# posgraph/coupe.DVSG

Measured on AMD Instinct MI355X. Metric: stabilized frames/sec (1280x720 RGB), higher is better.
Workload: dtype f32

## Files before the change

coupe/dvsg_amd/csrc/cnn_kernels.h:

```cpp
#pragma once
#include <type_traits>

#include "common.h"

namespace dvsg {

enum Precision { kF32 = 0, kF16 = 1, kF32S = 2, kF32X = 3 };
constexpr size_t elem_size(int prec) { return prec == kF16 ? 2 : 4; }
enum ConvMath { kMathF32, kMathF32S, kMathF32X, kMathF16Pairs, kMathF16Plain };
constexpr Precision storage_of(ConvMath m) { return m == kMathF32S ? kF32S : m == kMathF16Pairs || m == kMathF16Plain ? kF16 : kF32; }
constexpr ConvMath math_of(int prec, bool pairs) {
  return prec == kF16 ? (pairs ? kMathF16Pairs : kMathF16Plain) : prec == kF32S ? kMathF32S : prec == kF32X ? kMathF32X : kMathF32;
}
constexpr size_t elem_size(ConvMath m) { return elem_size((int)storage_of(m)); }
static_assert(storage_of(kMathF32) == kF32 && storage_of(kMathF32X) == kF32 && storage_of(kMathF32S) == kF32S &&
              storage_of(kMathF16Pairs) == kF16 && storage_of(kMathF16Plain) == kF16, "ConvMath -> storage format");
static_assert(math_of(kF32, false) == kMathF32 && math_of(kF32, true) == kMathF32 && math_of(kF32S, false) == kMathF32S &&
              math_of(kF32S, true) == kMathF32S && math_of(kF32X, false) == kMathF32X && math_of(kF32X, true) == kMathF32X &&
              math_of(kF16, true) == kMathF16Pairs && math_of(kF16, false) == kMathF16Plain, "(Precision, pairs) -> ConvMath");
static_assert(elem_size(kMathF32) == 4 && elem_size(kMathF32S) == 4 && elem_size(kMathF32X) == 4 &&
              elem_size(kMathF16Pairs) == 2 && elem_size(kMathF16Plain) == 2, "ConvMath -> bytes per tensor element");

struct ConvWeights {
  const void *rows = nullptr, *packed = nullptr, *packed_a = nullptr, *packed_h = nullptr;
// ... 86 lines not shown
  const int rec[6] = {family, nw, to, src, bands, quads};
  for (int i = 0; i < 6; ++i) g_last_root_kernel[i] = rec[i];
}
enum Conv1SrcKind { kSrcWindow = 0, kSrcRingF32 = 1, kSrcRingU8 = 2 };
constexpr int kSrcAligned = 1;
constexpr int kSrcKindShift = 1;
constexpr int kSrcMasked = 8;
constexpr int conv1_src(int kind, bool aligned, bool masked) {
  return (kind << kSrcKindShift) | (aligned ? kSrcAligned : 0) | (masked ? kSrcMasked : 0);
}
struct Conv1Src {
  const void *base;
  const int *table;
  int n_pool;
  const float *mask = nullptr;
};
struct Conv1Weights {
  const float *f32;
  const _Float16 *f16;
  const _Float16 *pieces;
  const unsigned short *x3;
  const float *bias;
};
int launch_conv1(int out_prec, const Conv1Src &src, int src_kind, const Conv1Weights &wt, void *y, int B, int H, int W, int Ho,
                 int Wo, int cin, hipStream_t s);
int prepare_rootconv();
int prepare_root_band();

int launch_maxpool(int prec, const void *x, void *y, int B, int H, int W, int C, int Ho, int Wo, int pad_top,
                   int pad_left, hipStream_t s);

constexpr int kPoolSplits = 8;
int launch_avgpool_partial(int prec, const void *x, float *part, int B, int HW, int C, hipStream_t s);

int launch_f16_to_f32(const void *x, float *y, size_t n, hipStream_t s);
int launch_p_to_f32(const void *x, float *y, size_t n, hipStream_t s);
int launch_f32_to_p(const float *x, void *y, size_t n, hipStream_t s);

constexpr int kDenseSplits = 8;
int launch_dense(const float *xin, int s_in, const float *bias_in, float scale_in, int lrelu_in,
                 const float *W, float *out_part, int B, int K, int N, hipStream_t s);
int launch_dense_finalize(const float *part, int s_in, float scale, const float *bias, float *out, int B,
                          int N, hipStream_t s);

}
```

coupe/dvsg_amd/csrc/common.h:

```cpp
#pragma once
#include <hip/hip_runtime.h>

#include <cstdarg>
#include <cstdio>

#include "../../../include/dvsg_amd.h"

namespace dvsg {

char *error_buffer();
int fail(int status, const char *fmt, ...) __attribute__((format(printf, 2, 3)));

inline hipStream_t as_stream(void *s) { return reinterpret_cast<hipStream_t>(s); }

inline int check_launch(const char *what) {
  hipError_t e = hipGetLastError();
  if (e != hipSuccess) return fail(DVSG_ERR_HIP, "%s: %s", what, hipGetErrorString(e));
  return DVSG_OK;
}

#define DVSG_REQUIRE(cond, ...)                                  \
  do {                                                           \
    if (!(cond)) return ::dvsg::fail(DVSG_ERR_INVALID_ARG, __VA_ARGS__); \
  } while (0)
// ... 26 lines not shown
int tps_render_impl(const double *winv_cols, const float *coord, const float *F_t, const uint8_t *src, int B, int H, int W,
                    int P, int channel_flip, float *T, float *out_f32, uint8_t *out_u8, int u8_W, int u8_x0, void *stream,
                    const float *zoom = nullptr, int render_filter = DVSG_RENDER_BILINEAR ,
                    int render_border = DVSG_BORDER_BLACK ,
                    RenderShape shape = RenderShape() );
int tps_render_nv12_check(const float *F_t, const uint8_t *y, const uint8_t *uv, size_t pitch, size_t frame_stride, int n,
                          int H, int W, const float *T, const uint8_t *out_y, const uint8_t *out_uv, size_t out_pitch,
                          size_t out_frame_stride, const char *fn = "dvsg_tps_render_nv12");
int tps_render_p010_check(const uint8_t *y, const uint8_t *uv, size_t pitch, size_t frame_stride, int n, int W,
                          const uint8_t *out_y, const uint8_t *out_uv, size_t out_pitch, size_t out_frame_stride, const char *fn);
int tps_render_nv12_impl(const double *winv_cols, const float *coord, const float *F_t, const uint8_t *y, const uint8_t *uv,
                         size_t pitch, size_t frame_stride, int n, int H, int W, int P, float *T, uint8_t *out_y,
                         uint8_t *out_uv, size_t out_pitch, size_t out_frame_stride, void *stream,
                         const float *zoom = nullptr, int render_filter = DVSG_RENDER_BILINEAR,
                         int render_border = DVSG_BORDER_BLACK, RenderShape shape = RenderShape(),
                         int surface_format = DVSG_SURFACE_NV12);
int tps_coverage_impl(const char *fn, const float *coord, long coord_bstride, const float *T, const float *zoom, int B, int P,
                      int src_H, int src_W, int out_h, int out_w, int32_t *n_border, int32_t *key_min, void *workspace,
                      size_t workspace_bytes, void *stream);

struct DebugOptions {
  int conv_variant = 0;
  int conv1_variant = 0;
  int wide16_min_tiles = 128;
  int wide16_packed = 1;
  int wide16_arows = 1;
  int wide16_hreuse = 1;
  int fused_hreuse = 1;
  int fuse_conv = 1;
  int fuse_shortcut = 1;
  int concat_sc = 1;
  int x3_conv1 = 1;
  int x3_fuse = 3;
  int f16_split = 1;
  int f16_pair_mask = 0xFFFF;
  int flow_tiled = 1;
  int flow_rounds = 4;
  int warp_xcd = 0;
};
extern DebugOptions g_opt;

inline int ceil_div(long a, long b) { return (int)((a + b - 1) / b); }

__device__ __forceinline__ uint8_t to_u8(double x) {
  const double d = x * 255.0;
  return d >= 255.0 ? (uint8_t)255 : (d > 0.0 ? (uint8_t)(int)d : (uint8_t)0);
// ... 36 lines not shown
```

coupe/dvsg_amd/csrc/conv1_pool.hip:

```cpp
#include <cstdint>
#include <type_traits>
#include <utility>

#include "cnn_device.h"
#include "cnn_kernels.h"

namespace dvsg {
namespace {

constexpr int C1_TILE = 128;
constexpr int C1_SEG_PAD = 5488;
constexpr int C1_WELEMS = 64 * kConv1Ld;
constexpr int C1_LDC = 68;

template <int NT, int GROUPS, bool ALIGNED, bool MASKED = false>
struct Conv1Row {
  static constexpr bool kRing = false;
  typedef float floatx4_u __attribute__((ext_vector_type(4), aligned(4)));
  floatx4 nmean[GROUPS];
  long idx[GROUPS];
  unsigned col_ok, full;
  bool fast;
  struct Data {
    floatx4 reg[GROUPS];
// ... 448 lines not shown
  __syncthreads();
  TO *yrow = y + (((size_t)b * Ho + ho) * Wo + wo0) * 64 + 4 * (tid & 15);
  conv1_tile_out<NT / 16>(Cs, conv1_tile_bias(bias, tid), tid, wo0, Wo,
                          [&](int row, float4 v) __attribute__((always_inline)) { store4(yrow + (size_t)row * 64, v); });
#ifdef DVSG_STAMPS
  if (tid == 0 && blockIdx.x < 65536) {
    unsigned long long *o = g_c1_stamps + (size_t)blockIdx.x * 8;
    const unsigned long long t_end = C1_STAMP();
    o[0] = st[0]; o[1] = st[1]; o[2] = st[2]; o[3] = st[3]; o[4] = st[4];
    o[5] = t_loop_end - t_begin;
    o[6] = t_end - t_begin;
    o[7] = __builtin_amdgcn_s_memrealtime() - r_begin;
  }
#endif
}

constexpr int RB_NT = 512;
constexpr int RB_IN4 = (C1_SEG_PAD / 4 + RB_NT - 1) / RB_NT;
constexpr int RB_WLOADS = (C1_WELEMS / 4 + RB_NT - 1) / RB_NT;
constexpr int RB_SLOTS = 3;
constexpr size_t RB_LDS = sizeof(float) * (size_t)(2 * C1_WELEMS + RB_SLOTS * C1_SEG_PAD);
static_assert(RB_LDS <= 160 * 1024, "the band kernel's LDS must fit a CU");

template <int SRC>
__global__ __launch_bounds__(RB_NT) __attribute__((amdgpu_waves_per_eu(2, 2)))
void root_band_kernel(const Conv1Src src, const float *__restrict__ wt1, const float *__restrict__ bias,
                      float *__restrict__ y, int H, int W, int Ho, int Wo, int wtiles, int bands, int ppb, int nbig) {
  constexpr int NT = RB_NT, MI = 2;
  static_assert(C1_TILE * C1_LDC <= C1_WELEMS, "epilogue tile must fit in a weight buffer");
  extern __shared__ __attribute__((aligned(16))) float rb_lds[];
  float *const w_s = rb_lds;
  float *const in_s = rb_lds + 2 * C1_WELEMS;
  const int tid = threadIdx.x;
  const int lane = tid & 63, wave = tid >> 6;
  const int wr = wave >> 2, wm = (wave >> 1) & 1, wn = wave & 1;
  const int r = lane & 31, h = lane >> 5;

  const Conv1Tile tile = conv1_tile(wtiles, bands);
  const int b = tile.b, band = tile.ho, wo0 = tile.wo0;
  const int pairs = (Ho + 1) / 2;
  const int p0 = band * ppb - (band > nbig ? band - nbig : 0);
  const int p1 = min(p0 + (band < nbig ? ppb : ppb - 1), pairs);
  if (p0 >= p1) return;

#ifdef DVSG_STAMPS
  unsigned long long st[8] = {0, 0, 0, 0, 0, 0, 0, 0};
  const unsigned long long t_begin = C1_STAMP(), r_begin = __builtin_amdgcn_s_memrealtime();
#endif
  typedef typename Conv1RowSel<NT, RB_IN4, SRC>::type Row;
  Row row;
  row.init(src, tid, b, wo0, H, W, C1_SEG_PAD);
  if constexpr (Row::kRing) {
    for (int e = tid; e < RB_SLOTS * C1_SEG_PAD; e += NT) in_s[e] = 0.f;
    __syncthreads();
  }
  typename Row::Data rd[3];
  floatx4 w_reg[RB_WLOADS];
  auto load_w = [&](int kh) __attribute__((always_inline)) {
    const floatx4 *wsrc = reinterpret_cast<const floatx4 *>(wt1 + (size_t)kh * C1_WELEMS);
#pragma unroll
    for (int i = 0; i < RB_WLOADS; ++i) {
      const int q = tid + NT * i;
      w_reg[i] = wsrc[q < C1_WELEMS / 4 ? q : 0];
    }
  };
  auto put_w = [&](int i, float *dst) __attribute__((always_inline)) {
    const int q = tid + NT * i;
    if (q < C1_WELEMS / 4) reinterpret_cast<floatx4 *>(dst)[q] = w_reg[i];
  };
  auto put_row = [&](const typename Row::Data &d, float *slot) __attribute__((always_inline)) {
    if constexpr (Row::kRing) {
      row.scatter(d, [&](int e, float v) __attribute__((always_inline)) { slot[e] = v; });
    } else {
#pragma unroll
      for (int i = 0; i < RB_IN4; ++i) {
        const int q = tid + NT * i;
        const floatx4 v = row.scaled(d, i);
        if (q < C1_SEG_PAD / 4) reinterpret_cast<floatx4 *>(slot)[q] = v;
      }
    }
  };
  auto load_first = [&](int ho_) __attribute__((always_inline)) {
#pragma unroll
    for (int i = 0; i < 3; ++i) row.load(rd[i], 2 * ho_ - 3 + i);
    load_w(0);
  };
#ifdef DVSG_STAMPS
  st[0] = C1_STAMP() - t_begin;
#endif
  load_first(2 * p0);

  for (int p = p0; p < p1; ++p) {
    const int ho = 2 * p;
#ifdef DVSG_STAMPS
    const unsigned long long f0 = C1_STAMP();
#endif
#pragma unroll
    for (int i = 0; i < RB_WLOADS; ++i) put_w(i, w_s);
#pragma unroll
    for (int i = 0; i < 3; ++i) {
      __builtin_amdgcn_sched_barrier(0);
      put_row(rd[i], in_s + i * C1_SEG_PAD);
    }
    __builtin_amdgcn_sched_barrier(0);
    floatx16 acc[MI], acc2[MI];
#pragma unroll
    for (int mi = 0; mi < MI; ++mi)
#pragma unroll
      for (int q = 0; q < 16; ++q) acc[mi][q] = acc2[mi][q] = 0.f;
#ifdef DVSG_STAMPS
    const unsigned long long f1 = C1_STAMP();
    __syncthreads();
    st[2] += f1 - f0;
    st[3] += C1_STAMP() - f1;
#else
    __syncthreads();
#endif

    int s_up = 0;
    for (int t = 0; t < 7; ++t) {
#ifdef DVSG_STAMPS
      const unsigned long long s3 = C1_STAMP();
#endif
      if (t < 6) {
        row.load(rd[0], 2 * ho + t);
        load_w(t + 1);
      }
#ifdef DVSG_STAMPS
      st[4] += C1_STAMP() - s3;
#endif
      __builtin_amdgcn_sched_barrier(0);
      const int s_lo = s_up == 0 ? 2 : s_up - 1;
      const float *a0 = in_s + (wr ? s_lo : s_up) * C1_SEG_PAD + 2 * kConv1Cin * (wm * 32 * MI + r) + 2 * h;
      const float *bp = w_s + (t & 1) * C1_WELEMS + (wn * 32 + r) * kConv1Ld + 2 * h;
      float *w_next = w_s + ((t + 1) & 1) * C1_WELEMS;
      constexpr int STEPS = kConv1Kpad / 4, PAIRS = (STEPS + 1) / 2;
      constexpr int WPUT0 = PAIRS / 2;
      float2 va[2][2][MI], vb[2][2];
      auto read_pair = [&](int slot, int g) __attribute__((always_inline)) {
#pragma unroll
        for (int j = 0; j < 2; ++j) {
          if (2 * g + j >= STEPS) break;
#pragma unroll
          for (int mi = 0; mi < MI; ++mi)
            va[slot][j][mi] = *reinterpret_cast<const float2 *>(a0 + mi * (2 * kConv1Cin * 32) + 4 * (2 * g + j));
          vb[slot][j] = *reinterpret_cast<const float2 *>(bp + 4 * (2 * g + j));
        }
      };
      read_pair(0, 0);
#pragma unroll
      for (int g = 0; g < PAIRS; ++g) {
        if (g + 1 < PAIRS) read_pair((g + 1) & 1, g + 1);
        if (g >= WPUT0 && g < WPUT0 + RB_WLOADS) put_w(g - WPUT0, w_next);
        __builtin_amdgcn_sched_barrier(0);
#pragma unroll
        for (int j = 0; j < 2; ++j) {
          if (2 * g + j >= STEPS) break;
#pragma unroll
          for (int mi = 0; mi < MI; ++mi) acc[mi] = mfma32(va[g & 1][j][mi].x, vb[g & 1][j].x, acc[mi]);
#pragma unroll
          for (int mi = 0; mi < MI; ++mi) acc2[mi] = mfma32(va[g & 1][j][mi].y, vb[g & 1][j].y, acc2[mi]);
        }
        __builtin_amdgcn_sched_barrier(0);
      }
      if (t < 6) {
#ifdef DVSG_STAMPS
        const unsigned long long s0 = C1_STAMP();
        __syncthreads();
        const unsigned long long s1 = C1_STAMP();
        put_row(rd[0], in_s + s_up * C1_SEG_PAD);
        const unsigned long long s2 = C1_STAMP();
        __syncthreads();
        st[1] += s1 - s0;
        st[2] += s2 - s1;
        st[3] += C1_STAMP() - s2;
#else
        __syncthreads();
        put_row(rd[0], in_s + s_up * C1_SEG_PAD);
        __syncthreads();
#endif
      }
      s_up = s_up == 2 ? 0 : s_up + 1;
    }

#ifdef DVSG_STAMPS
    const unsigned long long e0 = C1_STAMP();
#endif
    __syncthreads();
    float *Cs = w_s + wr * C1_WELEMS;
#pragma unroll
    for (int mi = 0; mi < MI; ++mi)
      C1_TILE_PUT(Cs, wm * 32 * MI + mi * 32, wn * 32, acc[mi][q] + acc2[mi][q]);
    __builtin_amdgcn_sched_barrier(0);
    if (p + 1 < p1) load_first(ho + 2);
    int tid_e = tid;
    asm volatile("" : "+v"(tid_e));
    const float4 b4 = conv1_tile_bias(bias, tid_e);
    __builtin_amdgcn_sched_barrier(0);
    __syncthreads();
#pragma unroll
    for (int j = 0; j < 2; ++j) {
      if (ho + j >= Ho) break;
      float *yrow = y + (((size_t)b * Ho + ho + j) * Wo + wo0) * 64 + 4 * (tid_e & 15);
      conv1_tile_out<NT / 16>(w_s + j * C1_WELEMS, b4, tid_e, wo0, Wo,
                              [&](int row_, float4 v) __attribute__((always_inline)) { store4(yrow + (size_t)row_ * 64, v); });
    }
    __syncthreads();
#ifdef DVSG_STAMPS
    st[5] += C1_STAMP() - e0;
#endif
  }
#ifdef DVSG_STAMPS
  if (tid == 0 && blockIdx.x < 65536) {
    unsigned long long *o = g_c1_stamps + (size_t)blockIdx.x * 8;
    o[0] = st[0]; o[1] = st[1]; o[2] = st[2]; o[3] = st[3]; o[4] = st[4]; o[5] = st[5];
    o[6] = C1_STAMP() - t_begin;
    o[7] = __builtin_amdgcn_s_memrealtime() - r_begin;
  }
#endif
}

struct PPieces {};

constexpr int rootconv_seg(int cin) { return C1_RING_PX * rootconv_pitch(cin) + 4; }
constexpr int rootconv_wstage(int cin) { return 64 * rootconv_ld(cin) > C1_TILE * C1_LDC ? 64 * rootconv_ld(cin) : C1_TILE * C1_LDC; }
constexpr size_t rootconv_lds_bytes(int cin) { return sizeof(float) * (size_t)(rootconv_wstage(cin) + rootconv_seg(cin)); }
static_assert(rootconv_lds_bytes(3 * kRootMaxFrames) <= 160 * 1024, "the largest window must fit one workgroup's LDS");

template <typename TO, int SRC>
__global__ __launch_bounds__(256)
void rootconv_kernel(const Conv1Src src, const float *__restrict__ wt1, const float *__restrict__ bias, void *__restrict__ y,
                     int H, int W, int Ho, int Wo, int wtiles, int cin) {
  constexpr int NT = 256, MI = 2;
  constexpr int kKind = SRC >> kSrcKindShift & 3;
  constexpr bool kMasked = (SRC & kSrcMasked) != 0;
  static_assert(SRC >= 0 && SRC < 16 && kKind <= kSrcRingU8, "no such conv1 source");
  extern __shared__ __attribute__((aligned(16))) float rc_lds[];
  const int S = cin / 3, pitch = rootconv_pitch(cin), ldw = rootconv_ld(cin), steps = rootconv_kpad(cin) / 4;
  const int welems = 64 * ldw, seg = rootconv_seg(cin);
  float *w_s = rc_lds;
  float *in_s = rc_lds + rootconv_wstage(cin);
  const int tid = threadIdx.x;
// ... 1088 lines not shown
}

template <int S>
using SrcC = std::integral_constant<int, S>;
template <bool MASKED_TOO, typename F>
bool with_conv1_src(int src, F &&f) {
  auto is = [&](auto c) { return src == c && (f(c), true); };
  if (is(SrcC<conv1_src(kSrcWindow, false, false)>{}) || is(SrcC<conv1_src(kSrcWindow, true, false)>{}) ||
      is(SrcC<conv1_src(kSrcRingF32, false, false)>{}) || is(SrcC<conv1_src(kSrcRingF32, true, false)>{}) ||
      is(SrcC<conv1_src(kSrcRingU8, false, false)>{}) || is(SrcC<conv1_src(kSrcRingU8, true, false)>{}))
    return true;
  if constexpr (MASKED_TOO)
    return is(SrcC<conv1_src(kSrcWindow, false, true)>{}) || is(SrcC<conv1_src(kSrcWindow, true, true)>{}) ||
           is(SrcC<conv1_src(kSrcRingF32, false, true)>{}) || is(SrcC<conv1_src(kSrcRingF32, true, true)>{}) ||
           is(SrcC<conv1_src(kSrcRingU8, false, true)>{}) || is(SrcC<conv1_src(kSrcRingU8, true, true)>{});
  return false;
}

}

int g_last_root_kernel[kRootKernelFields] = {-1, -1, -1, -1, -1, -1, -1, -1, -1};

int launch_conv1(int out_prec, const Conv1Src &src, int src_kind, const Conv1Weights &wt, void *y, int B, int H, int W, int Ho,
                 int Wo, int cin, hipStream_t s) {
  const float *const wt1 = wt.f32, *const bias = wt.bias;
  const _Float16 *const wt1h = wt.f16, *const wt1s = wt.pieces;
  const unsigned short *const wt1x = wt.x3;
  DVSG_REQUIRE(cin % 3 == 0 && cin >= 3 && cin <= 3 * kRootMaxFrames, "conv1: %d input channels", cin);
  const int wtiles = ceil_div(Wo, C1_TILE);
  const long blocks = (long)wtiles * Ho * B;
  DVSG_REQUIRE(blocks > 0 && blocks < (1L << 31), "conv1: grid of %ld workgroups out of range", blocks);
  DVSG_REQUIRE((long)W * cin < (1L << 31), "conv1: input row too long");
  DVSG_REQUIRE(src_kind == kSrcWindow || (src.table && src.n_pool > 0), "conv1: a frame ring needs its index table");
  const double in_bytes = src_kind == kSrcRingU8 ? 1.0 : 4.0;
  ProfScope prof(kClsConv1, s, 2.0 * (double)B * Ho * Wo * 64 * 49 * cin,
                 in_bytes * (double)B * H * W * cin + (double)elem_size(out_prec) * B * Ho * Wo * 64);
  const dim3 grid((unsigned)blocks);
  const bool aligned = W % 4 == 0 && reinterpret_cast<uintptr_t>(src.base) % (src_kind == kSrcRingU8 ? 4 : 16) == 0;
  const int SRC = conv1_src(src_kind, aligned, src.mask != nullptr);
  if (cin != kConv1Cin) {
    DVSG_REQUIRE(wt1, "conv1: no float32 weight image");
    const int to = out_prec == kF16 ? 1 : (out_prec == kF32S ? 2 : 0);
    const size_t lds = rootconv_lds_bytes(cin);
    const bool known = with_conv1_src<true>(SRC, [&](auto src_c) {
      constexpr int S = decltype(src_c)::value;
      record_conv1_kernel(6, 4, to, S);
      if (to == 1)
// ... 48 lines not shown
    });
  } else if (out_prec == kF16 && wt1h && variant != 2) {
    const int hpairs = (Ho + 1) / 2;
    const dim3 pgrid((unsigned)((long)wtiles * hpairs * B));
    legal = with_conv1_src<true>(SRC, [&](auto src_c) {
      constexpr int S = decltype(src_c)::value;
      record_conv1_kernel(2, -1, 1, S);
      hipLaunchKernelGGL((conv1_f16_pair_kernel<_Float16, S>), pgrid, dim3(256), 0, s, src, wt1h, bias,
                         static_cast<_Float16 *>(y), H, W, Ho, Wo, wtiles, hpairs);
    });
  } else if (out_prec == kF16) {
    DVSG_REQUIRE(src_kind == kSrcWindow && !src.mask, "conv1: conv1_variant 2 takes an unmasked window tensor");
    record_conv1_kernel(0, 4, 1, 0);
    hipLaunchKernelGGL((conv1_kernel<4, _Float16, 0>), grid, dim3(256), 0, s, src, wt1, bias, static_cast<_Float16 *>(y), H, W,
                       Ho, Wo, wtiles);
  } else if (!src.mask && (variant == 6 || (variant == 0 && root_bands(B, Ho, wtiles, nullptr, nullptr) > 0))) {
    int ppb = 0, nbig = 0;
    int bands = root_bands(B, Ho, wtiles, &ppb, &nbig);
    if (variant == 6) {
      ppb = 3;
      bands = nbig = ((Ho + 1) / 2 + ppb - 1) / ppb;
    }
    const dim3 bgrid((unsigned)((long)wtiles * bands * B));
    legal = with_conv1_src<false>(SRC, [&](auto src_c) {
      constexpr int S = decltype(src_c)::value;
      record_conv1_kernel(7, 8, 0, S, bands, ppb);
      hipLaunchKernelGGL((root_band_kernel<S>), bgrid, dim3(RB_NT), RB_LDS, s, src, wt1, bias, static_cast<float *>(y), H, W, Ho,
                         Wo, wtiles, bands, ppb, nbig);
    });
  } else if (variant != 0 && variant != 7 && src_kind == kSrcWindow && !src.mask) {
    record_conv1_kernel(0, 8, 0, 0);
    hipLaunchKernelGGL((conv1_kernel<8, float, 0>), grid, dim3(512), 0, s, src, wt1, bias, static_cast<float *>(y), H, W, Ho,
                       Wo, wtiles);
  } else {
    legal = with_conv1_src<true>(SRC, [&](auto src_c) {
      constexpr int S = decltype(src_c)::value;
      record_conv1_kernel(0, 4, 0, S);
      hipLaunchKernelGGL((conv1_kernel<4, float, S>), grid, dim3(256), 0, s, src, wt1, bias, static_cast<float *>(y), H, W, Ho, Wo,
                         wtiles);
    });
  }
  DVSG_REQUIRE(legal, "conv1: no kernel for source %d", SRC);
  return check_launch("conv1_kernel");
}

int prepare_rootconv() {
  const int bytes = (int)rootconv_lds_bytes(3 * kRootMaxFrames);
  hipError_t err = hipSuccess;
  auto raise = [&](const void *fn) {
    const hipError_t e = hipFuncSetAttribute(fn, hipFuncAttributeMaxDynamicSharedMemorySize, bytes);
    if (err == hipSuccess) err = e;
  };
  for (int src = 0; src < 16; ++src)
    with_conv1_src<true>(src, [&](auto src_c) {
      constexpr int S = decltype(src_c)::value;
      raise(reinterpret_cast<const void *>(&rootconv_kernel<float, S>));
      raise(reinterpret_cast<const void *>(&rootconv_kernel<_Float16, S>));
      raise(reinterpret_cast<const void *>(&rootconv_kernel<PPieces, S>));
    });
  DVSG_HIP(err);
  return DVSG_OK;
}

int prepare_root_band() {
  hipError_t err = hipSuccess;
  for (int src = 0; src < 16; ++src)
    with_conv1_src<false>(src, [&](auto src_c) {
      constexpr int S = decltype(src_c)::value;
      const hipError_t e = hipFuncSetAttribute(reinterpret_cast<const void *>(&root_band_kernel<S>),
                                               hipFuncAttributeMaxDynamicSharedMemorySize, (int)RB_LDS);
      if (err == hipSuccess) err = e;
    });
  DVSG_HIP(err);
  return DVSG_OK;
}

#ifdef DVSG_STAMPS
extern "C" int dvsg_debug_read_conv1_stamps(void *host, size_t bytes) {
  return hipMemcpyFromSymbol(host, HIP_SYMBOL(g_c1_stamps), bytes) == hipSuccess ? 0 : -3;
}
#endif

int launch_maxpool(int prec, const void *x, void *y, int B, int H, int W, int C, int Ho, int Wo, int pad_top,
                   int pad_left, hipStream_t s) {
  DVSG_REQUIRE(C % 4 == 0 && (prec != kF32S || C % 32 == 0), "maxpool: C=%d must be a multiple of 4 (32 in the f32s format)", C);
  const size_t total = (size_t)B * Ho * Wo * (C / 4);
  const size_t want = (total + 255) / 256;
  DVSG_REQUIRE(want < (1u << 31), "maxpool: %zu blocks do not fit a grid", want);
  const int blocks = (int)want;
  ProfScope prof(kClsMaxpool, s, 0.0, (double)elem_size(prec) * C * ((double)B * H * W + (double)B * Ho * Wo));
  g_last_root_kernel[kRootMaxpool] = prec == kF32S ? 3 : (prec == kF16 ? (C % 8 == 0 ? 2 : 1) : 0);
  if (prec == kF32S)
    hipLaunchKernelGGL(maxpool_p_kernel, dim3(blocks), dim3(256), 0, s, x, y, H, W, C / 4, Ho, Wo, pad_top, pad_left, total);
  else if (prec == kF16 && C % 8 == 0) {
    const size_t total8 = total / 2;
    hipLaunchKernelGGL(maxpool_h8_kernel, dim3((unsigned)((total8 + 255) / 256)), dim3(256), 0, s, static_cast<const _Float16 *>(x),
                       static_cast<_Float16 *>(y), H, W, C / 8, Ho, Wo, pad_top, pad_left, total8);
  } else if (prec == kF16)
    hipLaunchKernelGGL(maxpool_kernel<_Float16>, dim3(blocks), dim3(256), 0, s, static_cast<const _Float16 *>(x),
                       static_cast<_Float16 *>(y), H, W, C / 4, Ho, Wo, pad_top, pad_left, total);
  else
    hipLaunchKernelGGL(maxpool_kernel<float>, dim3(blocks), dim3(256), 0, s, static_cast<const float *>(x),
                       static_cast<float *>(y), H, W, C / 4, Ho, Wo, pad_top, pad_left, total);
  return check_launch("maxpool_kernel");
}

}
```

coupe/dvsg_amd/csrc/locnet.hip:

```cpp
#include <atomic>
#include <cmath>
#include <cstring>
#include <map>
#include <string>
#include <vector>

#include "cnn_kernels.h"

namespace dvsg {
namespace {

constexpr float kBnEps = 1e-5f;
const char *kPrefix = "stabNet/localizationNet/";

struct HostArray {
  const float *data;
  int nd;
  int64_t dims[4];
  size_t size() const {
    size_t n = 1;
    for (int i = 0; i < nd; ++i) n *= (size_t)dims[i];
    return n;
  }
};
// ... 420 lines not shown
    } else if (act == kF32S) {
      if (int rc = launch_p_to_f32(x, act_out, n, s)) return rc;
    } else {
      DVSG_HIP(hipMemcpyAsync(act_out, x, n * sizeof(float), hipMemcpyDeviceToDevice, s));
    }
    act_dims[0] = h; act_dims[1] = w; act_dims[2] = c;
    return 1;
  };
#define DVSG_TAP(stage, x, h, w, c)            \
  do {                                         \
    int t_ = tap(stage, x, h, w, c);           \
    if (t_ < 0) return t_;                     \
    if (t_ > 0) return DVSG_OK;                \
  } while (0)
#define DVSG_RUN(call)             \
  do {                             \
    if (int rc_ = (call)) return rc_; \
  } while (0)

  DVSG_RUN(launch_zero_tickets(ws.splitk_counters, (size_t)kMaxConvLaunches * kSplitKMaxTiles, s));
  ConvScratch scratch{ws};
  const bool fuse_allowed = g_opt.fuse_conv != 0 && calib == nullptr;
  reset_root_kernel();
  {
  MarkerRange mr("dvsg/conv1");
  DVSG_RUN(launch_conv1(precision == kF32X && g_opt.x3_conv1 ? kF32X : act, src, src_kind, net->conv1.conv1_images(), ws.bufA, B, H, W,
                        d.H1, d.W1, net->c_in, s));
  }
  DVSG_TAP(0, ws.bufA, d.H1, d.W1, 64);
  {
  MarkerRange mr("dvsg/pool1");
  DVSG_RUN(launch_maxpool(act, ws.bufA, ws.bufB, B, d.H1, d.W1, 64, d.Hp, d.Wp, d.pad_top, d.pad_left, s));
  }
  DVSG_TAP(1, ws.bufB, d.Hp, d.Wp, 64);

  char *X = ws.bufB, *Y = ws.bufA;
  int h = d.Hp, w = d.Wp;
  int stage = 2;
  int unit_in_block = 0, last_block = -1;
  for (const Unit &u : net->units) {
    unit_in_block = u.block == last_block ? unit_in_block + 1 : 1;
    last_block = u.block;
    char range_name[40];
    std::snprintf(range_name, sizeof(range_name), "dvsg/block%d/unit_%d", u.block + 1, unit_in_block);
    MarkerRange mr(range_name);
    const int ho = (h - 1) / u.stride + 1, wo = (w - 1) / u.stride + 1;
    ConvRes res{X, h, w, u.stride};
    auto math = [&](int kind) { return math_of(precision, f16_pairs(net, u.block, kind)); };
    const int calib_slot = 3 * (stage - 2);
    DVSG_RUN(calib_record(calib, calib_slot, X, (long)B * h * w, u.c1.cin, s));
    const bool x3_fused = precision == kF32X && g_opt.x3_fuse == 3;
    const bool x3_unfused = precision == kF32X && (g_opt.x3_fuse == 0 || (g_opt.x3_fuse == 1 && !u.has_shortcut));
    const bool fuse23 = fuse_allowed && !x3_unfused && conv_fusable(act, u.c2.cin, u.c2.cout, u.c3.cout, u.c2.ksize) &&
                        (act != kF16 || (f16_pairs(net, u.block, kKindC2) && f16_pairs(net, u.block, kKindC3) &&
                                         (!u.has_shortcut || f16_pairs(net, u.block, kKindSc))));
// ... 189 lines not shown
  f.B = B; f.H = H; f.W = W; f.Cin = Cin; f.Cout = Cout;
  f.Ho = (H - 1) / stride + 1; f.Wo = (W - 1) / stride + 1;
  f.stride = stride;
  f.res_H = (f.Ho - 1) * res_stride + 1; f.res_W = (f.Wo - 1) * res_stride + 1; f.res_stride = res_stride;
  if (sc_x) {
    f.res = nullptr;
    f.sc_x = sc_x; f.sc_wt = sc_wt; f.sc_bias = sc_bias;
    f.sc_cin = sc_cin;
  }
  return launch_conv3x3_1x1(f, as_stream(stream));
}

int opt_any(int v) { return v; }
int opt_flag(int v) { return v != 0; }
int opt_positive(int v) { return v > 0 ? v : 1; }
int opt_mask16(int v) { return v & 0xFFFF; }
constexpr struct {
  const char *name;
  int DebugOptions::*member;
  int (*normalise)(int);
} kDebugOptions[] = {
    {"conv_variant", &DebugOptions::conv_variant, opt_any},
    {"conv1_variant", &DebugOptions::conv1_variant, opt_any},
    {"wide16_min_tiles", &DebugOptions::wide16_min_tiles, opt_any},
    {"wide16_packed", &DebugOptions::wide16_packed, opt_any},
    {"wide16_arows", &DebugOptions::wide16_arows, opt_any},
    {"wide16_hreuse", &DebugOptions::wide16_hreuse, opt_any},
    {"fused_hreuse", &DebugOptions::fused_hreuse, opt_any},
    {"fuse_conv", &DebugOptions::fuse_conv, opt_any},
    {"fuse_shortcut", &DebugOptions::fuse_shortcut, opt_flag},
    {"concat_sc", &DebugOptions::concat_sc, opt_flag},
    {"x3_conv1", &DebugOptions::x3_conv1, opt_any},
    {"x3_fuse", &DebugOptions::x3_fuse, opt_any},
    {"f16_split", &DebugOptions::f16_split, opt_flag},
    {"f16_pair_mask", &DebugOptions::f16_pair_mask, opt_mask16},
    {"flow_tiled", &DebugOptions::flow_tiled, opt_any},
    {"flow_rounds", &DebugOptions::flow_rounds, opt_positive},
    {"warp_xcd", &DebugOptions::warp_xcd, opt_flag},
};

}
}

extern "C" {

int dvsg_locnet_create(int n_arrays, const char *const *names, const float *const *host_data, const int *ndims,
// ... 652 lines not shown
```

Baseline: 744.7.

## Fuse root maxpool into conv1 band kernel with seam fix-up pass

Adds a pooling variant of the root band conv1 kernel. It computes the 3x3/2 maxpool directly from the conv tile in LDS and carries partial row maxima across row pairs in an extra LDS buffer. It writes to the full conv output only the seam taps needed at tile and band boundaries. A small seam kernel then finishes the pooled values that cross column tiles and bands, replacing the full maxpool pass. This is meant to avoid writing and re-reading the full conv1 activation, at the cost of more LDS per block and an extra small launch.

Result: faster. 752.2, median of 6 (+1.0%).

```diff
diff --git a/coupe/dvsg_amd/csrc/cnn_kernels.h b/coupe/dvsg_amd/csrc/cnn_kernels.h
--- a/coupe/dvsg_amd/csrc/cnn_kernels.h
+++ b/coupe/dvsg_amd/csrc/cnn_kernels.h
@@ -132,8 +132,14 @@
   const unsigned short *x3;
   const float *bias;
 };
+struct RootPool {
+  void *pooled;
+  bool fused = false;
+  int bands = 0, ppb = 0, nbig = 0;
+};
 int launch_conv1(int out_prec, const Conv1Src &src, int src_kind, const Conv1Weights &wt, void *y, int B, int H, int W, int Ho,
-                 int Wo, int cin, hipStream_t s);
+                 int Wo, int cin, hipStream_t s, RootPool *pool = nullptr);
+int launch_root_pool_seams(const RootPool &pool, const void *conv_taps, int B, int Ho, int Wo, hipStream_t s);
 int prepare_rootconv();
 int prepare_root_band();
 
diff --git a/coupe/dvsg_amd/csrc/common.h b/coupe/dvsg_amd/csrc/common.h
--- a/coupe/dvsg_amd/csrc/common.h
+++ b/coupe/dvsg_amd/csrc/common.h
@@ -72,6 +72,7 @@
 struct DebugOptions {
   int conv_variant = 0;
   int conv1_variant = 0;
+  int root_pool = 0;
   int wide16_min_tiles = 128;
   int wide16_packed = 1;
   int wide16_arows = 1;
diff --git a/coupe/dvsg_amd/csrc/conv1_pool.hip b/coupe/dvsg_amd/csrc/conv1_pool.hip
--- a/coupe/dvsg_amd/csrc/conv1_pool.hip
+++ b/coupe/dvsg_amd/csrc/conv1_pool.hip
@@ -494,202 +494,73 @@
 constexpr size_t RB_LDS = sizeof(float) * (size_t)(2 * C1_WELEMS + RB_SLOTS * C1_SEG_PAD);
 static_assert(RB_LDS <= 160 * 1024, "the band kernel's LDS must fit a CU");
 
-template <int SRC>
-__global__ __launch_bounds__(RB_NT) __attribute__((amdgpu_waves_per_eu(2, 2)))
-void root_band_kernel(const Conv1Src src, const float *__restrict__ wt1, const float *__restrict__ bias,
-                      float *__restrict__ y, int H, int W, int Ho, int Wo, int wtiles, int bands, int ppb, int nbig) {
-  constexpr int NT = RB_NT, MI = 2;
-  static_assert(C1_TILE * C1_LDC <= C1_WELEMS, "epilogue tile must fit in a weight buffer");
-  extern __shared__ __attribute__((aligned(16))) float rb_lds[];
-  float *const w_s = rb_lds;
-  float *const in_s = rb_lds + 2 * C1_WELEMS;
-  const int tid = threadIdx.x;
-  const int lane = tid & 63, wave = tid >> 6;
-  const int wr = wave >> 2, wm = (wave >> 1) & 1, wn = wave & 1;
-  const int r = lane & 31, h = lane >> 5;
-
-  const Conv1Tile tile = conv1_tile(wtiles, bands);
-  const int b = tile.b, band = tile.ho, wo0 = tile.wo0;
-  const int pairs = (Ho + 1) / 2;
-  const int p0 = band * ppb - (band > nbig ? band - nbig : 0);
-  const int p1 = min(p0 + (band < nbig ? ppb : ppb - 1), pairs);
-  if (p0 >= p1) return;
-
-#ifdef DVSG_STAMPS
-  unsigned long long st[8] = {0, 0, 0, 0, 0, 0, 0, 0};
-  const unsigned long long t_begin = C1_STAMP(), r_begin = __builtin_amdgcn_s_memrealtime();
-#endif
-  typedef typename Conv1RowSel<NT, RB_IN4, SRC>::type Row;
-  Row row;
-  row.init(src, tid, b, wo0, H, W, C1_SEG_PAD);
-  if constexpr (Row::kRing) {
-    for (int e = tid; e < RB_SLOTS * C1_SEG_PAD; e += NT) in_s[e] = 0.f;
-    __syncthreads();
-  }
-  typename Row::Data rd[3];
-  floatx4 w_reg[RB_WLOADS];
-  auto load_w = [&](int kh) __attribute__((always_inline)) {
-    const floatx4 *wsrc = reinterpret_cast<const floatx4 *>(wt1 + (size_t)kh * C1_WELEMS);
-#pragma unroll
-    for (int i = 0; i < RB_WLOADS; ++i) {
-      const int q = tid + NT * i;
-      w_reg[i] = wsrc[q < C1_WELEMS / 4 ? q : 0];
-    }
+constexpr int RB_CARRY = 64 * 64;
+constexpr size_t RB_POOL_LDS = RB_LDS + sizeof(float) * RB_CARRY;
+static_assert(RB_POOL_LDS <= 160 * 1024, "the pooling band kernel's LDS must fit a CU");
+
+#define RB_KERNEL root_band_kernel
+#define RB_POOL 0
+#include "root_band_kernel.inc"
+#undef RB_KERNEL
+#undef RB_POOL
+#define RB_KERNEL root_band_pool_kernel
+#define RB_POOL 1
+#include "root_band_kernel.inc"
+#undef RB_KERNEL
+#undef RB_POOL
+
+__global__ __launch_bounds__(256) void root_pool_seams_kernel(const float *__restrict__ a, float *__restrict__ y, int Ho, int Wo,
+                                                             int ncs, int bands, int ppb, int nbig, size_t n_col,
+                                                             size_t total) {
+  const size_t e = (size_t)blockIdx.x * 256 + threadIdx.x;
+  if (e >= total) return;
+  const int Hp = Ho >> 1, Wp = Wo >> 1;
+  const int c4 = (int)(e & 15);
+  auto band_start = [&](int i) { return i * ppb - (i > nbig ? i - nbig : 0); };
+  int r, c;
+  size_t b;
+  bool col_seam, row_seam;
+  if (e < n_col) {
+    size_t t = e >> 4;
+    c = 64 * (int)(t % ncs) + 63;
+    t /= ncs;
+    r = (int)(t % Hp);
+    b = t / Hp;
+    const int p = r + 1, full = nbig * ppb;
+    const int i = p < full ? p / ppb : nbig + (p - full) / (ppb > 1 ? ppb - 1 : 1);
+    col_seam = true;
+    row_seam = p < Hp && i < bands && band_start(i) == p;
+  } else {
+    size_t t = (e - n_col) >> 4;
+    c = (int)(t % Wp);
+    t /= Wp;
+    r = band_start((int)(t % (bands - 1)) + 1) - 1;
+    b = t / (bands - 1);
+    if (r < 0 || r + 1 >= Hp) return;
+    if ((c & 63) == 63 && 2 * c + 2 < Wo) return;
+    col_seam = false;
+    row_seam = true;
+  }
+  float *const out = y + ((b * Hp + r) * Wp + c) * 64 + 4 * c4;
+  float4 m = load4(out);
+  auto take = [&](int hi, int wi) {
+    const float4 v = load4(a + ((b * Ho + hi) * Wo + wi) * 64 + 4 * c4);
+    m.x = fmaxf(m.x, v.x);
+    m.y = fmaxf(m.y, v.y);
+    m.z = fmaxf(m.z, v.z);
+    m.w = fmaxf(m.w, v.w);
   };
-  auto put_w = [&](int i, float *dst) __attribute__((always_inline)) {
-    const int q = tid + NT * i;
-    if (q < C1_WELEMS / 4) reinterpret_cast<floatx4 *>(dst)[q] = w_reg[i];
-  };
-  auto put_row = [&](const typename Row::Data &d, float *slot) __attribute__((always_inline)) {
-    if constexpr (Row::kRing) {
-      row.scatter(d, [&](int e, float v) __attribute__((always_inline)) { slot[e] = v; });
-    } else {
-#pragma unroll
-      for (int i = 0; i < RB_IN4; ++i) {
-        const int q = tid + NT * i;
-        const floatx4 v = row.scaled(d, i);
-        if (q < C1_SEG_PAD / 4) reinterpret_cast<floatx4 *>(slot)[q] = v;
-      }
-    }
-  };
-  auto load_first = [&](int ho_) __attribute__((always_inline)) {
-#pragma unroll
-    for (int i = 0; i < 3; ++i) row.load(rd[i], 2 * ho_ - 3 + i);
-    load_w(0);
-  };
-#ifdef DVSG_STAMPS
-  st[0] = C1_STAMP() - t_begin;
-#endif
-  load_first(2 * p0);
-
-  for (int p = p0; p < p1; ++p) {
-    const int ho = 2 * p;
-#ifdef DVSG_STAMPS
-    const unsigned long long f0 = C1_STAMP();
-#endif
-#pragma unroll
-    for (int i = 0; i < RB_WLOADS; ++i) put_w(i, w_s);
-#pragma unroll
-    for (int i = 0; i < 3; ++i) {
-      __builtin_amdgcn_sched_barrier(0);
-      put_row(rd[i], in_s + i * C1_SEG_PAD);
-    }
-    __builtin_amdgcn_sched_barrier(0);
-    floatx16 acc[MI], acc2[MI];
-#pragma unroll
-    for (int mi = 0; mi < MI; ++mi)
-#pragma unroll
-      for (int q = 0; q < 16; ++q) acc[mi][q] = acc2[mi][q] = 0.f;
-#ifdef DVSG_STAMPS
-    const unsigned long long f1 = C1_STAMP();
-    __syncthreads();
-    st[2] += f1 - f0;
-    st[3] += C1_STAMP() - f1;
-#else
-    __syncthreads();
-#endif
-
-    int s_up = 0;
-    for (int t = 0; t < 7; ++t) {
-#ifdef DVSG_STAMPS
-      const unsigned long long s3 = C1_STAMP();
-#endif
-      if (t < 6) {
-        row.load(rd[0], 2 * ho + t);
-        load_w(t + 1);
-      }
-#ifdef DVSG_STAMPS
-      st[4] += C1_STAMP() - s3;
-#endif
-      __builtin_amdgcn_sched_barrier(0);
-      const int s_lo = s_up == 0 ? 2 : s_up - 1;
-      const float *a0 = in_s + (wr ? s_lo : s_up) * C1_SEG_PAD + 2 * kConv1Cin * (wm * 32 * MI + r) + 2 * h;
-      const float *bp = w_s + (t & 1) * C1_WELEMS + (wn * 32 + r) * kConv1Ld + 2 * h;
-      float *w_next = w_s + ((t + 1) & 1) * C1_WELEMS;
-      constexpr int STEPS = kConv1Kpad / 4, PAIRS = (STEPS + 1) / 2;
-      constexpr int WPUT0 = PAIRS / 2;
-      float2 va[2][2][MI], vb[2][2];
-      auto read_pair = [&](int slot, int g) __attribute__((always_inline)) {
-#pragma unroll
-        for (int j = 0; j < 2; ++j) {
-          if (2 * g + j >= STEPS) break;
-#pragma unroll
-          for (int mi = 0; mi < MI; ++mi)
-            va[slot][j][mi] = *reinterpret_cast<const float2 *>(a0 + mi * (2 * kConv1Cin * 32) + 4 * (2 * g + j));
-          vb[slot][j] = *reinterpret_cast<const float2 *>(bp + 4 * (2 * g + j));
-        }
-      };
-      read_pair(0, 0);
-#pragma unroll
-      for (int g = 0; g < PAIRS; ++g) {
-        if (g + 1 < PAIRS) read_pair((g + 1) & 1, g + 1);
-        if (g >= WPUT0 && g < WPUT0 + RB_WLOADS) put_w(g - WPUT0, w_next);
-        __builtin_amdgcn_sched_barrier(0);
-#pragma unroll
-        for (int j = 0; j < 2; ++j) {
-          if (2 * g + j >= STEPS) break;
-#pragma unroll
-          for (int mi = 0; mi < MI; ++mi) acc[mi] = mfma32(va[g & 1][j][mi].x, vb[g & 1][j].x, acc[mi]);
-#pragma unroll
-          for (int mi = 0; mi < MI; ++mi) acc2[mi] = mfma32(va[g & 1][j][mi].y, vb[g & 1][j].y, acc2[mi]);
-        }
-        __builtin_amdgcn_sched_barrier(0);
-      }
-      if (t < 6) {
-#ifdef DVSG_STAMPS
-        const unsigned long long s0 = C1_STAMP();
-        __syncthreads();
-        const unsigned long long s1 = C1_STAMP();
-        put_row(rd[0], in_s + s_up * C1_SEG_PAD);
-        const unsigned long long s2 = C1_STAMP();
-        __syncthreads();
-        st[1] += s1 - s0;
-        st[2] += s2 - s1;
-        st[3] += C1_STAMP() - s2;
-#else
-        __syncthreads();
-        put_row(rd[0], in_s + s_up * C1_SEG_PAD);
-        __syncthreads();
-#endif
-      }
-      s_up = s_up == 2 ? 0 : s_up + 1;
-    }
-
-#ifdef DVSG_STAMPS
-    const unsigned long long e0 = C1_STAMP();
-#endif
-    __syncthreads();
-    float *Cs = w_s + wr * C1_WELEMS;
-#pragma unroll
-    for (int mi = 0; mi < MI; ++mi)
-      C1_TILE_PUT(Cs, wm * 32 * MI + mi * 32, wn * 32, acc[mi][q] + acc2[mi][q]);
-    __builtin_amdgcn_sched_barrier(0);
-    if (p + 1 < p1) load_first(ho + 2);
-    int tid_e = tid;
-    asm volatile("" : "+v"(tid_e));
-    const float4 b4 = conv1_tile_bias(bias, tid_e);
-    __builtin_amdgcn_sched_barrier(0);
-    __syncthreads();
-#pragma unroll
-    for (int j = 0; j < 2; ++j) {
-      if (ho + j >= Ho) break;
-      float *yrow = y + (((size_t)b * Ho + ho + j) * Wo + wo0) * 64 + 4 * (tid_e & 15);
-      conv1_tile_out<NT / 16>(w_s + j * C1_WELEMS, b4, tid_e, wo0, Wo,
-                              [&](int row_, float4 v) __attribute__((always_inline)) { store4(yrow + (size_t)row_ * 64, v); });
-    }
-    __syncthreads();
-#ifdef DVSG_STAMPS
-    st[5] += C1_STAMP() - e0;
-#endif
-  }
-#ifdef DVSG_STAMPS
-  if (tid == 0 && blockIdx.x < 65536) {
-    unsigned long long *o = g_c1_stamps + (size_t)blockIdx.x * 8;
-    o[0] = st[0]; o[1] = st[1]; o[2] = st[2]; o[3] = st[3]; o[4] = st[4]; o[5] = st[5];
-    o[6] = C1_STAMP() - t_begin;
-    o[7] = __builtin_amdgcn_s_memrealtime() - r_begin;
-  }
-#endif
+  if (col_seam) {
+#pragma unroll
+    for (int i = 0; i < 3; ++i)
+      if (2 * r + i < Ho) take(2 * r + i, 2 * c + 2);
+  }
+  if (row_seam) {
+#pragma unroll
+    for (int j = 0; j < 3; ++j)
+      if (2 * c + j < Wo && !(col_seam && j == 2)) take(2 * r + 2, 2 * c + j);
+  }
+  store4(out, m);
 }
 
 struct PPieces {};
@@ -1824,7 +1695,8 @@
 int g_last_root_kernel[kRootKernelFields] = {-1, -1, -1, -1, -1, -1, -1, -1, -1};
 
 int launch_conv1(int out_prec, const Conv1Src &src, int src_kind, const Conv1Weights &wt, void *y, int B, int H, int W, int Ho,
-                 int Wo, int cin, hipStream_t s) {
+                 int Wo, int cin, hipStream_t s, RootPool *pool) {
+  if (pool) pool->fused = false;
   const float *const wt1 = wt.f32, *const bias = wt.bias;
   const _Float16 *const wt1h = wt.f16, *const wt1s = wt.pieces;
   const unsigned short *const wt1x = wt.x3;
@@ -1919,11 +1791,22 @@
       bands = nbig = ((Ho + 1) / 2 + ppb - 1) / ppb;
     }
     const dim3 bgrid((unsigned)((long)wtiles * bands * B));
+    const bool fuse = pool && Ho % 2 == 0 && Wo % 2 == 0 && (g_opt.root_pool == 2 || (g_opt.root_pool == 0 && variant == 0));
+    if (fuse) {
+      pool->fused = true;
+      pool->bands = bands;
+      pool->ppb = ppb;
+      pool->nbig = nbig;
+    }
     legal = with_conv1_src<false>(SRC, [&](auto src_c) {
       constexpr int S = decltype(src_c)::value;
       record_conv1_kernel(7, 8, 0, S, bands, ppb);
-      hipLaunchKernelGGL((root_band_kernel<S>), bgrid, dim3(RB_NT), RB_LDS, s, src, wt1, bias, static_cast<float *>(y), H, W, Ho,
-                         Wo, wtiles, bands, ppb, nbig);
+      if (fuse)
+        hipLaunchKernelGGL((root_band_pool_kernel<S>), bgrid, dim3(RB_NT), RB_POOL_LDS, s, src, wt1, bias, static_cast<float *>(y),
+                           static_cast<float *>(pool->pooled), H, W, Ho, Wo, wtiles, bands, ppb, nbig);
+      else
+        hipLaunchKernelGGL((root_band_kernel<S>), bgrid, dim3(RB_NT), RB_LDS, s, src, wt1, bias, static_cast<float *>(y), H, W, Ho,
+                           Wo, wtiles, bands, ppb, nbig);
     });
   } else if (variant != 0 && variant != 7 && src_kind == kSrcWindow && !src.mask) {
     record_conv1_kernel(0, 8, 0, 0);
@@ -1967,6 +1850,9 @@
       const hipError_t e = hipFuncSetAttribute(reinterpret_cast<const void *>(&root_band_kernel<S>),
                                                hipFuncAttributeMaxDynamicSharedMemorySize, (int)RB_LDS);
       if (err == hipSuccess) err = e;
+      const hipError_t ep = hipFuncSetAttribute(reinterpret_cast<const void *>(&root_band_pool_kernel<S>),
+                                                hipFuncAttributeMaxDynamicSharedMemorySize, (int)RB_POOL_LDS);
+      if (err == hipSuccess) err = ep;
     });
   DVSG_HIP(err);
   return DVSG_OK;
@@ -2002,4 +1888,18 @@
   return check_launch("maxpool_kernel");
 }
 
-}
+int launch_root_pool_seams(const RootPool &pool, const void *conv_taps, int B, int Ho, int Wo, hipStream_t s) {
+  DVSG_REQUIRE(pool.fused && Ho % 2 == 0 && Wo % 2 == 0 && pool.bands >= 1, "root pool seams: no fused root launch to finish");
+  const int Hp = Ho / 2, Wp = Wo / 2, ncs = ceil_div(Wo, C1_TILE) - 1;
+  const size_t n_col = (size_t)B * Hp * ncs * 16, total = n_col + (size_t)B * (pool.bands - 1) * Wp * 16;
+  g_last_root_kernel[kRootMaxpool] = 4;
+  if (total == 0) return DVSG_OK;
+  const size_t want = (total + 255) / 256;
+  DVSG_REQUIRE(want < (1u << 31), "root pool seams: %zu blocks do not fit a grid", want);
+  ProfScope prof(kClsMaxpool, s, 0.0, 4.0 * 4.0 * (double)total * 5.0);
+  hipLaunchKernelGGL(root_pool_seams_kernel, dim3((unsigned)want), dim3(256), 0, s, static_cast<const float *>(conv_taps),
+                     static_cast<float *>(pool.pooled), Ho, Wo, ncs, pool.bands, pool.ppb, pool.nbig, n_col, total);
+  return check_launch("root_pool_seams_kernel");
+}
+
+}
diff --git a/coupe/dvsg_amd/csrc/locnet.hip b/coupe/dvsg_amd/csrc/locnet.hip
--- a/coupe/dvsg_amd/csrc/locnet.hip
+++ b/coupe/dvsg_amd/csrc/locnet.hip
@@ -466,15 +466,21 @@
   ConvScratch scratch{ws};
   const bool fuse_allowed = g_opt.fuse_conv != 0 && calib == nullptr;
   reset_root_kernel();
+  RootPool root_pool{ws.bufB};
+  const bool pool_in_conv1 = precision == kF32 && stop_stage != 0 && d.pad_top == 0 && d.pad_left == 0 && d.H1 % 2 == 0 &&
+                             d.W1 % 2 == 0 && g_opt.root_pool != 1;
   {
   MarkerRange mr("dvsg/conv1");
   DVSG_RUN(launch_conv1(precision == kF32X && g_opt.x3_conv1 ? kF32X : act, src, src_kind, net->conv1.conv1_images(), ws.bufA, B, H, W,
-                        d.H1, d.W1, net->c_in, s));
+                        d.H1, d.W1, net->c_in, s, pool_in_conv1 ? &root_pool : nullptr));
   }
   DVSG_TAP(0, ws.bufA, d.H1, d.W1, 64);
   {
   MarkerRange mr("dvsg/pool1");
-  DVSG_RUN(launch_maxpool(act, ws.bufA, ws.bufB, B, d.H1, d.W1, 64, d.Hp, d.Wp, d.pad_top, d.pad_left, s));
+  if (root_pool.fused)
+    DVSG_RUN(launch_root_pool_seams(root_pool, ws.bufA, B, d.H1, d.W1, s));
+  else
+    DVSG_RUN(launch_maxpool(act, ws.bufA, ws.bufB, B, d.H1, d.W1, 64, d.Hp, d.Wp, d.pad_top, d.pad_left, s));
   }
   DVSG_TAP(1, ws.bufB, d.Hp, d.Wp, 64);
 
@@ -710,6 +716,7 @@
 } kDebugOptions[] = {
     {"conv_variant", &DebugOptions::conv_variant, opt_any},
     {"conv1_variant", &DebugOptions::conv1_variant, opt_any},
+    {"root_pool", &DebugOptions::root_pool, opt_any},
     {"wide16_min_tiles", &DebugOptions::wide16_min_tiles, opt_any},
     {"wide16_packed", &DebugOptions::wide16_packed, opt_any},
     {"wide16_arows", &DebugOptions::wide16_arows, opt_any},
diff --git a/coupe/dvsg_amd/csrc/root_band_kernel.inc b/coupe/dvsg_amd/csrc/root_band_kernel.inc
--- /dev/null
+++ b/coupe/dvsg_amd/csrc/root_band_kernel.inc
@@ -0,0 +1,251 @@
+template <int SRC>
+__global__ __launch_bounds__(RB_NT) __attribute__((amdgpu_waves_per_eu(2, 2)))
+void RB_KERNEL(const Conv1Src src, const float *__restrict__ wt1, const float *__restrict__ bias,
+#if RB_POOL
+               float *__restrict__ y, float *__restrict__ pooled, int H, int W, int Ho, int Wo, int wtiles, int bands, int ppb, int nbig) {
+#else
+               float *__restrict__ y, int H, int W, int Ho, int Wo, int wtiles, int bands, int ppb, int nbig) {
+#endif
+  constexpr int NT = RB_NT, MI = 2;
+  static_assert(C1_TILE * C1_LDC <= C1_WELEMS, "epilogue tile must fit in a weight buffer");
+  extern __shared__ __attribute__((aligned(16))) float rb_lds[];
+  float *const w_s = rb_lds;
+  float *const in_s = rb_lds + 2 * C1_WELEMS;
+  const int tid = threadIdx.x;
+  const int lane = tid & 63, wave = tid >> 6;
+  const int wr = wave >> 2, wm = (wave >> 1) & 1, wn = wave & 1;
+  const int r = lane & 31, h = lane >> 5;
+
+  const Conv1Tile tile = conv1_tile(wtiles, bands);
+  const int b = tile.b, band = tile.ho, wo0 = tile.wo0;
+  const int pairs = (Ho + 1) / 2;
+  const int p0 = band * ppb - (band > nbig ? band - nbig : 0);
+  const int p1 = min(p0 + (band < nbig ? ppb : ppb - 1), pairs);
+  if (p0 >= p1) return;
+
+#ifdef DVSG_STAMPS
+  unsigned long long st[8] = {0, 0, 0, 0, 0, 0, 0, 0};
+  const unsigned long long t_begin = C1_STAMP(), r_begin = __builtin_amdgcn_s_memrealtime();
+#endif
+  typedef typename Conv1RowSel<NT, RB_IN4, SRC>::type Row;
+  Row row;
+  row.init(src, tid, b, wo0, H, W, C1_SEG_PAD);
+  if constexpr (Row::kRing) {
+    for (int e = tid; e < RB_SLOTS * C1_SEG_PAD; e += NT) in_s[e] = 0.f;
+    __syncthreads();
+  }
+  typename Row::Data rd[3];
+  floatx4 w_reg[RB_WLOADS];
+  auto load_w = [&](int kh) __attribute__((always_inline)) {
+    const floatx4 *wsrc = reinterpret_cast<const floatx4 *>(wt1 + (size_t)kh * C1_WELEMS);
+#pragma unroll
+    for (int i = 0; i < RB_WLOADS; ++i) {
+      const int q = tid + NT * i;
+      w_reg[i] = wsrc[q < C1_WELEMS / 4 ? q : 0];
+    }
+  };
+  auto put_w = [&](int i, float *dst) __attribute__((always_inline)) {
+    const int q = tid + NT * i;
+    if (q < C1_WELEMS / 4) reinterpret_cast<floatx4 *>(dst)[q] = w_reg[i];
+  };
+  auto put_row = [&](const typename Row::Data &d, float *slot) __attribute__((always_inline)) {
+    if constexpr (Row::kRing) {
+      row.scatter(d, [&](int e, float v) __attribute__((always_inline)) { slot[e] = v; });
+    } else {
+#pragma unroll
+      for (int i = 0; i < RB_IN4; ++i) {
+        const int q = tid + NT * i;
+        const floatx4 v = row.scaled(d, i);
+        if (q < C1_SEG_PAD / 4) reinterpret_cast<floatx4 *>(slot)[q] = v;
+      }
+    }
+  };
+  auto load_first = [&](int ho_) __attribute__((always_inline)) {
+#pragma unroll
+    for (int i = 0; i < 3; ++i) row.load(rd[i], 2 * ho_ - 3 + i);
+    load_w(0);
+  };
+#ifdef DVSG_STAMPS
+  st[0] = C1_STAMP() - t_begin;
+#endif
+  load_first(2 * p0);
+
+  for (int p = p0; p < p1; ++p) {
+    const int ho = 2 * p;
+#ifdef DVSG_STAMPS
+    const unsigned long long f0 = C1_STAMP();
+#endif
+#pragma unroll
+    for (int i = 0; i < RB_WLOADS; ++i) put_w(i, w_s);
+#pragma unroll
+    for (int i = 0; i < 3; ++i) {
+      __builtin_amdgcn_sched_barrier(0);
+      put_row(rd[i], in_s + i * C1_SEG_PAD);
+    }
+    __builtin_amdgcn_sched_barrier(0);
+    floatx16 acc[MI], acc2[MI];
+#pragma unroll
+    for (int mi = 0; mi < MI; ++mi)
+#pragma unroll
+      for (int q = 0; q < 16; ++q) acc[mi][q] = acc2[mi][q] = 0.f;
+#ifdef DVSG_STAMPS
+    const unsigned long long f1 = C1_STAMP();
+    __syncthreads();
+    st[2] += f1 - f0;
+    st[3] += C1_STAMP() - f1;
+#else
+    __syncthreads();
+#endif
+
+    int s_up = 0;
+    for (int t = 0; t < 7; ++t) {
+#ifdef DVSG_STAMPS
+      const unsigned long long s3 = C1_STAMP();
+#endif
+      if (t < 6) {
+        row.load(rd[0], 2 * ho + t);
+        load_w(t + 1);
+      }
+#ifdef DVSG_STAMPS
+      st[4] += C1_STAMP() - s3;
+#endif
+      __builtin_amdgcn_sched_barrier(0);
+      const int s_lo = s_up == 0 ? 2 : s_up - 1;
+      const float *a0 = in_s + (wr ? s_lo : s_up) * C1_SEG_PAD + 2 * kConv1Cin * (wm * 32 * MI + r) + 2 * h;
+      const float *bp = w_s + (t & 1) * C1_WELEMS + (wn * 32 + r) * kConv1Ld + 2 * h;
+      float *w_next = w_s + ((t + 1) & 1) * C1_WELEMS;
+      constexpr int STEPS = kConv1Kpad / 4, PAIRS = (STEPS + 1) / 2;
+      constexpr int WPUT0 = PAIRS / 2;
+      float2 va[2][2][MI], vb[2][2];
+      auto read_pair = [&](int slot, int g) __attribute__((always_inline)) {
+#pragma unroll
+        for (int j = 0; j < 2; ++j) {
+          if (2 * g + j >= STEPS) break;
+#pragma unroll
+          for (int mi = 0; mi < MI; ++mi)
+            va[slot][j][mi] = *reinterpret_cast<const float2 *>(a0 + mi * (2 * kConv1Cin * 32) + 4 * (2 * g + j));
+          vb[slot][j] = *reinterpret_cast<const float2 *>(bp + 4 * (2 * g + j));
+        }
+      };
+      read_pair(0, 0);
+#pragma unroll
+      for (int g = 0; g < PAIRS; ++g) {
+        if (g + 1 < PAIRS) read_pair((g + 1) & 1, g + 1);
+        if (g >= WPUT0 && g < WPUT0 + RB_WLOADS) put_w(g - WPUT0, w_next);
+        __builtin_amdgcn_sched_barrier(0);
+#pragma unroll
+        for (int j = 0; j < 2; ++j) {
+          if (2 * g + j >= STEPS) break;
+#pragma unroll
+          for (int mi = 0; mi < MI; ++mi) acc[mi] = mfma32(va[g & 1][j][mi].x, vb[g & 1][j].x, acc[mi]);
+#pragma unroll
+          for (int mi = 0; mi < MI; ++mi) acc2[mi] = mfma32(va[g & 1][j][mi].y, vb[g & 1][j].y, acc2[mi]);
+        }
+        __builtin_amdgcn_sched_barrier(0);
+      }
+      if (t < 6) {
+#ifdef DVSG_STAMPS
+        const unsigned long long s0 = C1_STAMP();
+        __syncthreads();
+        const unsigned long long s1 = C1_STAMP();
+        put_row(rd[0], in_s + s_up * C1_SEG_PAD);
+        const unsigned long long s2 = C1_STAMP();
+        __syncthreads();
+        st[1] += s1 - s0;
+        st[2] += s2 - s1;
+        st[3] += C1_STAMP() - s2;
+#else
+        __syncthreads();
+        put_row(rd[0], in_s + s_up * C1_SEG_PAD);
+        __syncthreads();
+#endif
+      }
+      s_up = s_up == 2 ? 0 : s_up + 1;
+    }
+
+#ifdef DVSG_STAMPS
+    const unsigned long long e0 = C1_STAMP();
+#endif
+    __syncthreads();
+    float *Cs = w_s + wr * C1_WELEMS;
+#pragma unroll
+    for (int mi = 0; mi < MI; ++mi)
+      C1_TILE_PUT(Cs, wm * 32 * MI + mi * 32, wn * 32, acc[mi][q] + acc2[mi][q]);
+    __builtin_amdgcn_sched_barrier(0);
+    if (p + 1 < p1) load_first(ho + 2);
+    int tid_e = tid;
+    asm volatile("" : "+v"(tid_e));
+    const float4 b4 = conv1_tile_bias(bias, tid_e);
+    __builtin_amdgcn_sched_barrier(0);
+    __syncthreads();
+#if RB_POOL
+    {
+      const int col4 = tid_e & 15;
+      const int nv = min(C1_TILE, Wo - wo0);
+      const int Hp = Ho >> 1, Wp = Wo >> 1;
+      auto tap = [&](int j, int px) __attribute__((always_inline)) {
+        float4 v = *reinterpret_cast<const float4 *>(w_s + j * C1_WELEMS + px * C1_LDC + 4 * col4);
+        v.x = fmaxf(v.x + b4.x, 0.f);
+        v.y = fmaxf(v.y + b4.y, 0.f);
+        v.z = fmaxf(v.z + b4.z, 0.f);
+        v.w = fmaxf(v.w + b4.w, 0.f);
+        return v;
+      };
+      auto max4 = [](float4 a, float4 c) __attribute__((always_inline)) {
+        return make_float4(fmaxf(a.x, c.x), fmaxf(a.y, c.y), fmaxf(a.z, c.z), fmaxf(a.w, c.w));
+      };
+      float *const carry_s = rb_lds + 2 * C1_WELEMS + RB_SLOTS * C1_SEG_PAD;
+      float *const prow = pooled + (((size_t)b * Hp + p) * Wp + (wo0 >> 1)) * 64 + 4 * col4;
+#pragma unroll
+      for (int k = 0; k < 2; ++k) {
+        const int lc = (tid_e >> 4) + 32 * k;
+        if (2 * lc >= nv) break;
+        const bool third = 2 * lc + 2 < nv;
+        float4 hu = make_float4(-INFINITY, -INFINITY, -INFINITY, -INFINITY), hl = hu;
+#pragma unroll
+        for (int i = 0; i < 3; ++i) {
+          if (i == 2 && !third) break;
+          hu = max4(hu, tap(0, 2 * lc + i));
+          hl = max4(hl, tap(1, 2 * lc + i));
+        }
+        float4 *const cp = reinterpret_cast<float4 *>(carry_s + lc * 64 + 4 * col4);
+        if (p > p0) store4(prow - (size_t)Wp * 64 + (size_t)lc * 64, max4(*cp, hu));
+        const float4 c = max4(hu, hl);
+        if (p + 1 < p1)
+          *cp = c;
+        else
+          store4(prow + (size_t)lc * 64, c);
+      }
+      if (wo0 > 0 && tid_e < 32) {
+        const int j = tid_e >> 4;
+        store4(y + (((size_t)b * Ho + ho + j) * Wo + wo0) * 64 + 4 * col4, tap(j, 0));
+      }
+      if (p == p0 && p0 > 0) {
+        float *yrow = y + (((size_t)b * Ho + ho) * Wo + wo0) * 64 + 4 * col4;
+        conv1_tile_out<NT / 16>(w_s, b4, tid_e, wo0, Wo,
+                                [&](int row_, float4 v) __attribute__((always_inline)) { store4(yrow + (size_t)row_ * 64, v); });
+      }
+    }
+#else
+#pragma unroll
+    for (int j = 0; j < 2; ++j) {
+      if (ho + j >= Ho) break;
+      float *yrow = y + (((size_t)b * Ho + ho + j) * Wo + wo0) * 64 + 4 * (tid_e & 15);
+      conv1_tile_out<NT / 16>(w_s + j * C1_WELEMS, b4, tid_e, wo0, Wo,
+                              [&](int row_, float4 v) __attribute__((always_inline)) { store4(yrow + (size_t)row_ * 64, v); });
+    }
+#endif
+    __syncthreads();
+#ifdef DVSG_STAMPS
+    st[5] += C1_STAMP() - e0;
+#endif
+  }
+#ifdef DVSG_STAMPS
+  if (tid == 0 && blockIdx.x < 65536) {
+    unsigned long long *o = g_c1_stamps + (size_t)blockIdx.x * 8;
+    o[0] = st[0]; o[1] = st[1]; o[2] = st[2]; o[3] = st[3]; o[4] = st[4]; o[5] = st[5];
+    o[6] = C1_STAMP() - t_begin;
+    o[7] = __builtin_amdgcn_s_memrealtime() - r_begin;
+  }
+#endif
+}
```
